# nyu-dl/MultimodalGame

Measured on AMD Instinct MI355X. Metric: exchange-steps/sec (whole node), 30-class Adaptive max_exchange=10 bs=64, higher is better.
Workload: dtype f32

## Files before the change

### multimodalgame_amd/csrc/kernels_bwd.h

```cpp
#pragma once
#include <type_traits>
#include "device_utils.h"
#include "layout.h"

namespace mmg {

template <bool CC = false>
__device__ __forceinline__ float combine_score(const float* part, size_t row, int npb, float b2) {
    float v = 0.f;
    if (npb <= 8) {
        float p[8];
#pragma unroll
        for (int j = 0; j < 8; ++j) p[j] = (j < npb) ? (CC ? __hip_atomic_load(&part[row * npb + j], __ATOMIC_RELAXED, __HIP_MEMORY_SCOPE_AGENT) : part[row * npb + j]) : 0.f;
#pragma unroll
        for (int j = 0; j < 8; ++j) v += p[j];
    } else {
        for (int j = 0; j < npb; ++j) v += part[row * npb + j];
    }
    return v + b2;
}

__host__ __device__ inline size_t partll_at(const Dims& d, int sen_side, size_t row, int npb) { return ((size_t)(sen_side ? 0 : 1) * d.T * d.B + row) * npb; }
__device__ __forceinline__ float combine_score_ll(const Dims& dm, const Tape& tp, int sen_side, size_t row, int npb, float b2, uint32_t epoch, bool need) {
    const size_t at = partll_at(dm, sen_side, row, npb);
// ... 396 lines not shown
            __syncthreads();
        }
        if (binary) {
            const float wh = (L - tp.bs[row]) * cw_z[t];
            for (int j = tid; j < W; j += nt) {
                const float v = bit_seed(tp.z[row * W + j], tp.pz[row * W + j], wh, ce_z[t]);
                s_dlz[j] = v; tp.dlz[row * W + j] = v;
            }
            __syncthreads();
            gemv_t<TU>(P.p[S_BIN_W], H, W, H, s_dlz, s_da, s_red, false);
            for (int i = tid; i < H; i += nt) {
                const float a = tp.a[row * H + i];
                const float v = s_da[i] * (1.f - a * a);
                s_dpre[i] = v; tp.dpre[row * H + i] = v; s_dhx[i] += v;
            }
            __syncthreads();
            if (t == 0) {
                gemv_t<TU>(P.p[S_CODE_W], W, H, W, s_dpre, s_dc0, s_red, false);
                for (int j = tid; j < W; j += nt) tp.dc0[(size_t)b * W + j] = s_dc0[j];
            }
            const float dbs = lc.cb[t] * (tp.bs[row] - L), dbr = lc.cb[t] * (tp.br[row] - L);
            if (tid == 0) { tp.dbs[row] = dbs; tp.dbr[row] = dbr; }
        } else {
            for (int i = tid; i < W; i += nt) tp.dlz[row * W + i] = 0.f;
            for (int i = tid; i < H; i += nt) tp.dpre[row * H + i] = 0.f;
            if (tid == 0) { tp.dbs[row] = 0.f; tp.dbr[row] = 0.f; }
        }
        __syncthreads();
    }
    for (int i = tid; i < H; i += nt) tp.dhx[(size_t)b * H + i] = s_dhx[i];
    if (!binary) for (int j = tid; j < W; j += nt) tp.dc0[(size_t)b * W + j] = 0.f;
}

template <bool CC = false>
__device__ __forceinline__ void build_row_map(const Dims& dm, const Tape& tp) {
    const int lane = threadIdx.x & 63, B = dm.B, T = dm.T;
    int base = 0;
    for (int t = 0; t < T; ++t) {
        for (int b0 = 0; b0 < B; b0 += 64) {
            const int b = b0 + lane;
            const int tsb = CC ? __hip_atomic_load(&tp.tstar[min(b, B - 1)], __ATOMIC_RELAXED, __HIP_MEMORY_SCOPE_AGENT) : tp.tstar[min(b, B - 1)];
            const bool act = (b < B) && (t <= tsb);
            const unsigned long long m = __ballot(act);
            const int pos = base + __popcll(m & ((1ull << lane) - 1ull));
            if (act) tp.rmap[pos] = t * B + b;
            base += __popcll(m);
        }
    }
    if (lane == 0) tp.rcount[0] = base;
    for (int i = base + lane; i < T * B; i += 64) tp.rmap[i] = -1;
}

template <bool CC = false>
__device__ __forceinline__ void dC_class(const Dims& dm, const Params& P, const Tape& tp, int d, float* s_c, float* s_p) {
    auto ld = [](const float* p) { return CC ? __hip_atomic_load(p, __ATOMIC_RELAXED, __HIP_MEMORY_SCOPE_AGENT) : *p; };
    const int tid = threadIdx.x, R = dm.R, B = dm.B, D = dm.D;
    const int cols = R < 64 ? R : 64;
    const int groups = MMG_BLOCK / cols;
    const int g = tid / cols, rr = tid - g * cols;
    const float* w2 = P.p[R_Y2_W];
    for (int r0 = 0; r0 < R; r0 += cols) {
        const int r = r0 + rr;
        float dc0 = 0.f, dc1 = 0.f, py0 = 0.f, py1 = 0.f;
        if (g < groups && r < R) {
            const float cv = ld(&tp.Cd[(size_t)d * R + r]);
            for (int b = g; b < B; b += 16 * groups) {
                float yv[16], pv[16];
#pragma unroll
                for (int u = 0; u < 16; ++u) {
                    const int bb = b + u * groups;
                    const bool ok = bb < B;
                    yv[u] = ok ? ld(&tp.dy[(size_t)bb * D + d]) : 0.f;
                    pv[u] = ok ? ld(&tp.Astar[(size_t)bb * R + r]) + cv : 0.f;
                }
#pragma unroll
                for (int u = 0; u < 16; u += 2) {
                    if (pv[u] > 0.f) { dc0 += yv[u]; py0 = fmaf(yv[u], pv[u], py0); }
                    if (pv[u + 1] > 0.f) { dc1 += yv[u + 1]; py1 = fmaf(yv[u + 1], pv[u + 1], py1); }
                }
            }
        }
        s_c[tid] = (dc0 + dc1) * ((g < groups && r < R) ? w2[r] : 0.f);
        s_p[tid] = py0 + py1;
        __syncthreads();
        if (tid < cols && r0 + tid < R) {
            float a = 0.f, c = 0.f;
            for (int k = 0; k < groups; ++k) { a += s_c[k * cols + tid]; c += s_p[k * cols + tid]; }
            tp.dC[(size_t)d * R + r0 + tid] = a;
            tp.Py2[(size_t)d * R + r0 + tid] = c;
        }
        __syncthreads();
    }
}

__global__ __launch_bounds__(MMG_BLOCK) void k_dC(Dims dm, Params P, Tape tp) {
    __shared__ float s_c[MMG_BLOCK], s_p[MMG_BLOCK];
    dC_class(dm, P, tp, blockIdx.x, s_c, s_p);
}

enum { SRC_STATIC = 0, SRC_X = 1, SRC_DESC = 2 };
struct GemmJob { const float* A; const float* Bm; float* C; const float* vhid; const float* vw2;
                 int lda, ldb, ldc, rows, N, K, bmod, bsrc, tile_begin, tiles_k, compact, nsplit; };
struct ColJob { const float* src; float* dst; const float* scale; const float* vbeta; const float* vw2; const float* wrow;
                int ld, rows, cols, blk_begin, compact, special; };
#define MMG_MAX_GEMM 40
#define MMG_MAX_COL 40
struct NormPlan { int64_t begin[MMG_GN_BLOCKS], end[MMG_GN_BLOCKS]; int agent[MMG_GN_BLOCKS]; };
#define MMG_MAX_WBLOCKS 16384
struct JobTable {
    int n_gemm, n_col, gemm_tiles, gemm_blocks, col_blocks, special_block, special_job, pad2;
    GemmJob g[MMG_MAX_GEMM];
    ColJob c[MMG_MAX_COL];
    NormPlan np;
    int g_begin[64], c_begin[64];
    int n_wblocks;
    signed char wblock_agent[MMG_MAX_WBLOCKS];
};

__device__ __forceinline__ float4 load4_guard(const float* __restrict__ base_, size_t row_off, int col, int ncols, bool row_ok, bool vec_ok) {
    float4 v = make_float4(0.f, 0.f, 0.f, 0.f);
    if (!row_ok) return v;
    gfloat* p = as_global(base_) + row_off + col;
    if (vec_ok && col + 3 < ncols) return ldg4(p);
    if (col < ncols) v.x = p[0];
    if (col + 1 < ncols) v.y = p[1];
    if (col + 2 < ncols) v.z = p[2];
    if (col + 3 < ncols) v.w = p[3];
    return v;
}

struct WgHead { int gemm_tiles, n_wblocks, special_block, special_job; };

struct OptArgs {
    int optim_type, only_receiver, from_wgrad, bump_step, bump_mb;
    float lr;
    int64_t agent_begin[5];
    int64_t total;
};

struct WgOpt {
    OptArgs oa;
    float* params; float* state; const float* grads; float* gnll; float* coefll;
    uint32_t* counter; uint32_t* err_host;
};
#define MMG_COEF_REPL 64
__device__ __forceinline__ void opt_update_one(const OptArgs& oa, float* params, float* state, int64_t idx, float g, float coef,
                                               float w, float s1, float s2, uint32_t step) {
    const float gv = g * coef;
    if (oa.optim_type == MMG_OPT_RMSPROP) {
        const float sv = 0.99f * s1 + (1.f - 0.99f) * gv * gv;
        w -= oa.lr * gv / (sqrtf(sv) + 1e-8f);
        state[idx] = sv;
    } else if (oa.optim_type == MMG_OPT_ADAM) {
        const float b1 = 0.9f, b2 = 0.999f;
        const float bc1 = 1.f - powf(b1, (float)step), bc2s = sqrtf(1.f - powf(b2, (float)step));
        const float mv = s1 + (gv - s1) * (1.f - b1), vv = b2 * s2 + (1.f - b2) * gv * gv;
        w -= (oa.lr / bc1) * mv / (sqrtf(vv) / bc2s + 1e-8f);
        state[idx] = mv; state[oa.total + idx] = vv;
    } else {
        w -= oa.lr * gv;
    }
    params[idx] = w;
}
__device__ __forceinline__ float opt_wait_coef(const WgOpt& wo, int agent, uint32_t epoch, const uint32_t* sync) {
    unsigned long long u;
    for (int spins = 0;; ) {
        u = ld_ll(wo.coefll, (size_t)agent * MMG_COEF_REPL + (blockIdx.x & (MMG_COEF_REPL - 1)));
        if (ll_fresh(u, epoch)) break;
        __builtin_amdgcn_s_sleep(2);
        if (++spins > (1 << 20)) { __hip_atomic_store(const_cast<uint32_t*>(sync) + MMG_SYNC_ERR, 10u, __ATOMIC_RELAXED, __HIP_MEMORY_SCOPE_AGENT); return -1.f; }
    }
    return ll_value(u);
}

template <bool OPT>
__global__ __launch_bounds__(MMG_BLOCK) void k_wgrad(const JobTable* __restrict__ jt, const float* __restrict__ x,
                                                     const float* __restrict__ desc, float* __restrict__ part,
                                                     Dims dm, const double* __restrict__ stats, float* __restrict__ losses,
                                                     double* __restrict__ totals, const int* __restrict__ rmap,
                                                     const int* __restrict__ rcount, float* __restrict__ wpart, uint32_t* __restrict__ wcnt,
                                                     const uint32_t* __restrict__ sync, float* __restrict__ grad_tail, WgOpt wo, int gt_stride, WgHead hd
#ifdef MMG_TIMING
                                                     , long long* __restrict__ dbg2
#endif
                                                     ) {
    const int bid = (gt_stride > 0 && (int)blockIdx.x >= gt_stride) ? (int)blockIdx.x - gt_stride + hd.gemm_tiles : (int)blockIdx.x;
    const uint32_t oepoch = OPT ? wo.counter[3] + 1u : 0u;
    const uint32_t ostep = OPT ? wo.counter[1] + 1u : 0u;
    if (OPT && bid > hd.n_wblocks) {
        __shared__ float s_ss[4];
        const int agent = bid - hd.n_wblocks - 1;
        const int n = hd.n_wblocks;
        float ss = 0.f;
        for (int k0 = threadIdx.x; k0 < n; k0 += 8 * MMG_BLOCK) {
            unsigned long long u[8]; bool mine[8], any[8];
#pragma unroll
            for (int q = 0; q < 8; ++q) {
                const int k = k0 + q * MMG_BLOCK;
                mine[q] = (k < n) && ((int)jt->wblock_agent[min(k, n - 1)] == agent);
                any[q] = __any(mine[q]);
                u[q] = 0ull;
            }
            for (int spins = 0;; ) {
                bool fresh = true;
#pragma unroll
                for (int q = 0; q < 8; ++q)
                    if (any[q]) {
                        const unsigned long long v = ld_ll(wo.gnll, (size_t)min(k0 + q * MMG_BLOCK, n - 1));
                        if (mine[q]) { u[q] = v; fresh = fresh && ll_fresh(v, oepoch); }
                    }
                if (!__any(!fresh)) break;
                __builtin_amdgcn_s_sleep(1);
                if (++spins > (1 << 20)) { __hip_atomic_store(const_cast<uint32_t*>(sync) + MMG_SYNC_ERR, 11u, __ATOMIC_RELAXED, __HIP_MEMORY_SCOPE_AGENT); break; }
            }
#pragma unroll
            for (int q = 0; q < 8; ++q) ss += mine[q] ? ll_value(u[q]) : 0.f;
        }
        const float wsum = dpp_wave_sum(ss);
        if ((threadIdx.x & 63) == 0) s_ss[threadIdx.x >> 6] = wsum;
        __syncthreads();
        const uint32_t err = __hip_atomic_load(sync + MMG_SYNC_ERR, __ATOMIC_RELAXED, __HIP_MEMORY_SCOPE_AGENT);
        if (threadIdx.x < MMG_COEF_REPL + 1) {
            const float tot = (s_ss[0] + s_ss[1]) + (s_ss[2] + s_ss[3]);
            const float coef = 1.0f / (sqrtf(tot) + 1e-6f);
            if (threadIdx.x < MMG_COEF_REPL) st_ll(wo.coefll, (size_t)agent * MMG_COEF_REPL + threadIdx.x, err != 0u ? -1.f : (coef < 1.f ? coef : 1.f), oepoch);
            else st_ll(wo.coefll, (size_t)4 * MMG_COEF_REPL + agent, tot, oepoch);
        }
        return;
    }
#ifdef MMG_TIMING
    if (threadIdx.x == 0 && blockIdx.x < 4096) dbg2[2 * blockIdx.x] = (long long)wall_clock64();
#define MMG_WG_END() do { __syncthreads(); if (threadIdx.x == 0 && blockIdx.x < 4096) dbg2[2 * blockIdx.x + 1] = (long long)wall_clock64(); } while (0)
#else
#define MMG_WG_END() do {} while (0)
#endif
    constexpr int CH = 64;
    __shared__ __attribute__((aligned(16))) float s_a[2][CH][16];
    __shared__ __attribute__((aligned(16))) float s_b[2][CH][48];
    float (*s_acc)[16][33] = reinterpret_cast<float (*)[16][33]>(&s_b[0][0][0]);
    float* s_part = &s_b[0][0][0];
    __shared__ float s_red[8];
    if (bid == hd.special_block) {
        const ColJob& C = jt->c[hd.special_job];
        float* s_v = &s_b[0][0][0];
        const int Hh = C.ld, Wc = C.cols, nb = C.rows;
        const int p8 = threadIdx.x & 7, jj = threadIdx.x >> 3;
        float wreg[32];
        const bool wfast = (Hh == 256) && (Wc <= 32);
        if (wfast) {
#pragma unroll
            for (int i = 0; i < 32; ++i) wreg[i] = C.wrow[(size_t)(p8 + 8 * i) * Wc + min(jj, Wc - 1)];
        }
        for (int h0 = threadIdx.x; h0 < Hh; h0 += MMG_BLOCK) {
            float a0 = 0.f, a1 = 0.f, a2 = 0.f, a3 = 0.f;
            for (int b0 = 0; b0 < nb; b0 += 64) {
                float v[64];
#pragma unroll
                for (int u = 0; u < 64; ++u) v[u] = C.src[(size_t)min(b0 + u, nb - 1) * Hh + h0];
#pragma unroll
                for (int u = 0; u < 64; u += 4) {
                    a0 += (b0 + u < nb) ? v[u] : 0.f; a1 += (b0 + u + 1 < nb) ? v[u + 1] : 0.f;
                    a2 += (b0 + u + 2 < nb) ? v[u + 2] : 0.f; a3 += (b0 + u + 3 < nb) ? v[u + 3] : 0.f;
                }
            }
            s_v[h0] = (a0 + a1) + (a2 + a3);
        }
        __syncthreads();
        float sq = 0.f;
        for (int j0 = 0; j0 < Wc; j0 += MMG_BLOCK / 8) {
            const int j = j0 + jj;
            float acc = 0.f;
            if (wfast) {
#pragma unroll
                for (int i = 0; i < 32; ++i) acc = fmaf(wreg[i], s_v[p8 + 8 * i], acc);
            } else if (j < Wc) {
                for (int h0 = p8; h0 < Hh; h0 += 8) acc = fmaf(C.wrow[(size_t)h0 * Wc + j], s_v[h0], acc);
            }
            acc = dpp_group_sum<8>(acc);
            if (j < Wc && p8 == 0) { const float gsum = acc * C.scale[j]; C.dst[j] = gsum; sq = fmaf(gsum, gsum, sq); }
        }
        sq = block_sum(sq, s_red);
        if (threadIdx.x == 0) part[bid] = sq;
        if (OPT) {
            if (threadIdx.x == 0) st_ll(wo.gnll, bid, sq, oepoch);
#ifdef MMG_TIMING
        if (threadIdx.x == 0 && bid < 2000) dbg2[8192 + 4 * bid + 2] = (long long)wall_clock64();
#endif
#ifdef MMG_TIMING
            if (threadIdx.x == 0 && bid < 2000) dbg2[8192 + 4 * bid + 2] = (long long)wall_clock64();
#endif
            const float coef = opt_wait_coef(wo, jt->wblock_agent[bid], oepoch, sync);
            for (int j0 = 0; j0 < Wc && coef >= 0.f; j0 += MMG_BLOCK / 8) {
                const int j = j0 + jj;
                if (j < Wc && p8 == 0) {
                    const int64_t idx = (C.dst - wo.grads) + j;
                    opt_update_one(wo.oa, wo.params, wo.state, idx, C.dst[j], coef, wo.params[idx], wo.state[idx],
                                   wo.oa.optim_type == MMG_OPT_ADAM ? wo.state[wo.oa.total + idx] : 0.f, ostep);
                }
            }
        }
        MMG_WG_END();
        return;
    }
    constexpr int MAXMAP = 2048;
    __shared__ unsigned short s_map[MAXMAP];
    const bool use_map = rmap != nullptr;
    int nact = 0;
    if (use_map) {
        const int tb = dm.T * dm.B;
        for (int i2 = threadIdx.x; i2 < tb; i2 += MMG_BLOCK) s_map[i2] = (unsigned short)rmap[i2];
        nact = rcount[0];
    }
    const int lane = threadIdx.x & 63, wave = threadIdx.x >> 6;
    if (bid == hd.n_wblocks) {
        float* s_lc = &s_b[0][0][0];
        LossCoef lc; lc.cw = s_lc; lc.ce = s_lc + 3 * dm.T; lc.cb = s_lc + 6 * dm.T;
        loss_coefficients(dm, stats, lc, losses, totals, !OPT);
        if (threadIdx.x == 0) {
            grad_tail[0] = (__hip_atomic_load(sync + MMG_SYNC_ERR, __ATOMIC_RELAXED, __HIP_MEMORY_SCOPE_AGENT) != 0u) ? 1.f : 0.f;
            grad_tail[1] = (float)stats[stat_glob(dm.T, 0)];
            grad_tail[2] = (float)stats[stat_glob(dm.T, 1)];
            grad_tail[3] = 0.f;
        }
        if (OPT) {
            __shared__ float s_tot[4];
            if (threadIdx.x < 4) {
                unsigned long long u;
                for (int spins = 0;; ) {
                    u = ld_ll(wo.coefll, (size_t)4 * MMG_COEF_REPL + threadIdx.x);
                    if (ll_fresh(u, oepoch)) break;
                    __builtin_amdgcn_s_sleep(2);
                    if (++spins > (1 << 20)) { __hip_atomic_store(const_cast<uint32_t*>(sync) + MMG_SYNC_ERR, 11u, __ATOMIC_RELAXED, __HIP_MEMORY_SCOPE_AGENT); break; }
                }
                s_tot[threadIdx.x] = ll_value(u);
            }
            __syncthreads();
            if (threadIdx.x == 0) {
                bool bad = false;
#pragma unroll
                for (int a = 0; a < 4; ++a) bad = bad || !(s_tot[a] == s_tot[a]) || s_tot[a] > 3.0e38f;
                losses[0] = bad ? __builtin_nanf("") : (float)(-stats[stat_glob(dm.T, 0)] / (double)dm.Bg);
                const uint32_t err = __hip_atomic_load(sync + MMG_SYNC_ERR, __ATOMIC_RELAXED, __HIP_MEMORY_SCOPE_AGENT);
                if (wo.err_host && (err != 0u || *wo.err_host == 0u)) *wo.err_host = err;
                if (err == 0u) wo.counter[2] = ostep;
                if (wo.oa.bump_mb) { wo.counter[0] += 1u; wo.counter[3] += 1u; }
            }
        }
        return;
    }
    if (bid < hd.gemm_tiles) {
      __shared__ int s_arrived;
      for (int vt = bid; vt < hd.gemm_tiles; vt += (gt_stride > 0 ? gt_stride : hd.gemm_tiles)) {
        const int nwg = hd.gemm_tiles, xq = nwg >> 3, xr = nwg & 7;
        const int xcd = vt & 7, slot = vt >> 3;
        const int tile = (xcd < xr ? xcd * (xq + 1) : xr * (xq + 1) + (xcd - xr) * xq) + slot;
        const int j = __popcll(__ballot(jt->g_begin[lane] <= tile)) - 1;
        const GemmJob& G = jt->g[j];
        const int ns = G.nsplit > 1 ? G.nsplit : 1;
        const int lts = tile - G.tile_begin, sp = lts % ns, lt = lts / ns;
        const int tn = lt / G.tiles_k, tk = lt - tn * G.tiles_k;
        const int n0 = tn * 16, k0 = tk * 32;
        const int i = lane & 15, q = lane >> 4;
        const float* Bbase = (G.bsrc == SRC_X) ? x : (G.bsrc == SRC_DESC) ? desc : G.Bm;
        const bool virt = G.vhid != nullptr;
        const float* Abase = virt ? G.vhid : G.A;
        const bool cmp = use_map && G.compact;
        const int lda = G.lda, ldb = G.ldb, bmod = G.bmod, N = G.N, K = G.K;
        const bool ident0 = cmp && dm.B >= 64 && sp == 0;
        int rows = cmp ? 0 : G.rows;
        const bool veca = ((lda & 3) == 0) && ((((uintptr_t)Abase) & 15) == 0);
        const bool vecb = ((ldb & 3) == 0) && ((((uintptr_t)Bbase) & 15) == 0);
        const int la = threadIdx.x >> 2, lac = (threadIdx.x & 3) * 4;
        const int lb0 = threadIdx.x >> 3, lbc = (threadIdx.x & 7) * 4;
        float4 vw = make_float4(0.f, 0.f, 0.f, 0.f);
        if (virt) vw = load4_guard(G.vw2, 0, n0 + lac, N, true, false);
        int nchunks_all = 0, cps = 0, cbeg = 0, cend = 0, nchunks = 0, rows_end = 0, rlast = 0;
        auto set_rows = [&](int r) {
            rows = r;
            nchunks_all = (rows + CH - 1) / CH; cps = (nchunks_all + ns - 1) / ns;
            cbeg = sp * cps; cend = min(nchunks_all, cbeg + cps); nchunks = max(cend - cbeg, 0);
            rows_end = min(rows, cend * CH);
            rlast = rows - 1;
        };
        if (!cmp) set_rows(G.rows);
        constexpr int DEPTH = 3;
        f32x4 acc0 = {0.f, 0.f, 0.f, 0.f}, acc1 = {0.f, 0.f, 0.f, 0.f};
        const bool interior = veca && vecb && ((G.bsrc != SRC_X) || (k0 + 32 <= K));
        const int bmodv = bmod ? bmod : 0x7fffffff;
        const uint32_t bmagic = bmod > 1 ? (uint32_t)((0x100000000ull + (unsigned)bmod - 1ull) / (unsigned)bmod) : 0u;
        const bool bmod_one = bmod == 1;
        (void)bmodv;
        auto rowmod = [&](int r) -> int {
            const int q = (int)__umulhi((uint32_t)r, bmagic);
            const int m = r - q * bmod;
            return bmod_one ? 0 : (m < 0 ? m + bmod : m);
        };
        gfloat* const Ag = as_global(Abase);
        gfloat* const Bg = as_global(Bbase);
        gfloat* const betag = as_global(G.A);
        auto run = [&](auto virt_tag, auto cmp_tag, auto bmod_tag) {
            constexpr bool VIRT = decltype(virt_tag)::value, CMPJ = decltype(cmp_tag)::value, BMOD = decltype(bmod_tag)::value;
            float4 ra[DEPTH], rb0[DEPTH], rb1[DEPTH];
            float beta[DEPTH];
            const uint32_t acol = (uint32_t)(n0 + lac), bcol = (uint32_t)(k0 + lbc), ulda = (uint32_t)lda, uldb = (uint32_t)ldb;
            auto issue = [&](int rc_, int c0_, int c1_, int u) {
                ra[u] = ldg4(Ag + ((uint32_t)rc_ * ulda + acol));
                if (VIRT) beta[u] = betag[(uint32_t)rc_];
                rb0[u] = ldg4(Bg + ((uint32_t)(BMOD ? rowmod(c0_) : c0_) * uldb + bcol));
                rb1[u] = ldg4(Bg + ((uint32_t)(BMOD ? rowmod(c1_) : c1_) * uldb + bcol));
            };
            auto fetch = [&](int c, int u) {
                const int r_ = c * CH + la, r0_ = c * CH + lb0, r1_ = r0_ + 32;
                int rc_ = min(r_, rlast), c0_ = min(r0_, rlast), c1_ = min(r1_, rlast);
                if (CMPJ) { rc_ = s_map[rc_]; c0_ = s_map[c0_]; c1_ = s_map[c1_]; }
                issue(rc_, c0_, c1_, u);
            };
            if (!CMPJ) {
#pragma unroll
                for (int u = 0; u < DEPTH - 1; ++u) fetch(cbeg + u, u);
            } else if (ident0) issue(la, lb0, lb0 + 32, 0);
            if (use_map) __syncthreads();
#ifdef MMG_TIMING
            if (threadIdx.x == 0 && tile < 2000) dbg2[8192 + 4 * tile + 0] = (long long)wall_clock64();
#endif
            if (CMPJ) {
                set_rows(nact);
#pragma unroll
                for (int u = 0; u < DEPTH - 1; ++u) if (u > 0 || !ident0) fetch(cbeg + u, u);
            }
            const int nouter = (nchunks + DEPTH - 1) / DEPTH;
            for (int o = 0; o < nouter; ++o) {
#pragma unroll
                for (int u = 0; u < DEPTH; ++u) {
                    const int c = cbeg + o * DEPTH + u;
                    const int buf = (o * DEPTH + u) & 1;
                    const bool va = (c * CH + la) < rows_end;
                    float4 av = ra[u];
                    if (VIRT) {
                        av.x = av.x > 0.f ? beta[u] * vw.x : 0.f; av.y = av.y > 0.f ? beta[u] * vw.y : 0.f;
                        av.z = av.z > 0.f ? beta[u] * vw.z : 0.f; av.w = av.w > 0.f ? beta[u] * vw.w : 0.f;
                    }
                    const float ma = va ? 1.f : 0.f;
                    *reinterpret_cast<float4*>(&s_a[buf][la][lac]) = make_float4(av.x * ma, av.y * ma, av.z * ma, av.w * ma);
                    *reinterpret_cast<float4*>(&s_b[buf][lb0][lbc]) = rb0[u];
                    *reinterpret_cast<float4*>(&s_b[buf][lb0 + 32][lbc]) = rb1[u];
                    __syncthreads();
                    fetch(c + DEPTH - 1, (u + DEPTH - 1) % DEPTH);
#pragma unroll
                    for (int v = 0; v < 4; ++v) {
                        const int r = wave * 16 + v * 4 + q;
                        const float a = s_a[buf][r][i];
                        acc0 = mfma16(a, s_b[buf][r][i], acc0);
                        acc1 = mfma16(a, s_b[buf][r][16 + i], acc1);
                    }
                }
            }
        };
        auto run_b = [&](auto virt_tag, auto cmp_tag) {
            if (bmod != 0) run(virt_tag, cmp_tag, std::true_type{}); else run(virt_tag, cmp_tag, std::false_type{});
        };
        auto run_c = [&](auto virt_tag) { if (cmp) run_b(virt_tag, std::true_type{}); else run_b(virt_tag, std::false_type{}); };
        if (interior) {
            if (virt) run_c(std::true_type{}); else run_c(std::false_type{});
        } else {
            if (use_map) __syncthreads();
            if (cmp) set_rows(nact);
            for (int c = cbeg; c < cend; ++c) {
                const int buf = c & 1;
                const int rl = c * CH + la;
                const bool rv = rl < rows_end;
                const int r = cmp ? (int)s_map[min(rl, rlast)] : rl;
                float4 av = load4_guard(Abase, (size_t)(rv ? r : 0) * lda, n0 + lac, N, rv, veca);
                if (virt) {
                    const float be = rv ? betag[r] : 0.f;
                    av.x = av.x > 0.f ? be * vw.x : 0.f; av.y = av.y > 0.f ? be * vw.y : 0.f;
                    av.z = av.z > 0.f ? be * vw.z : 0.f; av.w = av.w > 0.f ? be * vw.w : 0.f;
                }
                const int r0l = c * CH + lb0, r1l = r0l + 32;
                const bool v0 = r0l < rows_end, v1 = r1l < rows_end;
                const int r0 = cmp ? (int)s_map[min(r0l, rlast)] : r0l, r1 = cmp ? (int)s_map[min(r1l, rlast)] : r1l;
                const int m0 = bmod ? (r0 % bmod) : r0, m1 = bmod ? (r1 % bmod) : r1;
                const float4 b0v = load4_guard(Bbase, (size_t)(v0 ? m0 : 0) * ldb, k0 + lbc, K, v0, vecb);
                const float4 b1v = load4_guard(Bbase, (size_t)(v1 ? m1 : 0) * ldb, k0 + lbc, K, v1, vecb);
                *reinterpret_cast<float4*>(&s_a[buf][la][lac]) = av;
                *reinterpret_cast<float4*>(&s_b[buf][lb0][lbc]) = b0v;
                *reinterpret_cast<float4*>(&s_b[buf][lb0 + 32][lbc]) = b1v;
                __syncthreads();
#pragma unroll
                for (int v = 0; v < 4; ++v) {
                    const int rr2 = wave * 16 + v * 4 + q;
                    const float a = s_a[buf][rr2][i];
                    acc0 = mfma16(a, s_b[buf][rr2][i], acc0);
                    acc1 = mfma16(a, s_b[buf][rr2][16 + i], acc1);
                }
            }
        }
        __syncthreads();
#ifdef MMG_TIMING
        if (threadIdx.x == 0 && tile < 2000) dbg2[8192 + 4 * tile + 1] = (long long)wall_clock64();
#endif
#pragma unroll
        for (int r = 0; r < 4; ++r) { s_acc[wave][q * 4 + r][i] = acc0[r]; s_acc[wave][q * 4 + r][16 + i] = acc1[r]; }
        __syncthreads();
        float sq = 0.f;
        float gv2[2]; int64_t gi2[2];
#pragma unroll
        for (int h2 = 0; h2 < 2; ++h2) {
            const int rr = threadIdx.x >> 4, cc = (threadIdx.x & 15) + 16 * h2;
            const int n = n0 + rr, k = k0 + cc;
            const float v = (s_acc[0][rr][cc] + s_acc[1][rr][cc]) + (s_acc[2][rr][cc] + s_acc[3][rr][cc]);
            gv2[h2] = v; gi2[h2] = -1;
            if (ns > 1) st_wt(&wpart[(size_t)tile * 512 + rr * 32 + cc], v);
            else if (n < N && k < K) {
                as_global_w(G.C)[(size_t)n * G.ldc + k] = v;
                sq = fmaf(v, v, sq);
                gi2[h2] = (G.C - wo.grads) + (int64_t)n * G.ldc + k;
            }
        }
        bool adds_up = false;
        if (ns > 1) {
            asm volatile("s_waitcnt vmcnt(0)" ::: "memory");
            __syncthreads();
            const int tile0 = tile - sp;
            if (threadIdx.x == 0) s_arrived = (int)__hip_atomic_fetch_add(wcnt + tile0, 1u, __ATOMIC_RELAXED, __HIP_MEMORY_SCOPE_AGENT);
            __syncthreads();
            adds_up = __builtin_amdgcn_readfirstlane(s_arrived) == ns - 1;
            if (adds_up) {
                if (threadIdx.x == 0) __hip_atomic_store(wcnt + tile0, 0u, __ATOMIC_RELAXED, __HIP_MEMORY_SCOPE_AGENT);
#pragma unroll
                for (int h2 = 0; h2 < 2; ++h2) {
                    const int rr = threadIdx.x >> 4, cc = (threadIdx.x & 15) + 16 * h2;
                    float v = 0.f;
                    for (int s0 = 0; s0 < ns; s0 += 8) {
                        float pv[8];
#pragma unroll
                        for (int u = 0; u < 8; ++u) pv[u] = ld_cc(&wpart[(size_t)(tile0 + min(s0 + u, ns - 1)) * 512 + rr * 32 + cc]);
#pragma unroll
                        for (int u = 0; u < 8; ++u) v += (s0 + u < ns) ? pv[u] : 0.f;
                    }
                    const int n = n0 + rr, k = k0 + cc;
                    if (n < N && k < K) { as_global_w(G.C)[(size_t)n * G.ldc + k] = v; sq = fmaf(v, v, sq); }
                }
            }
        }
        sq = block_sum(sq, s_red);
        if (threadIdx.x == 0) {
            if (ns == 1) part[tile] = sq;
            else {
                if (sp != 0) part[tile] = 0.f;
                if (adds_up) part[tile - sp] = sq;
            }
        }
        if (OPT) {
            if (threadIdx.x == 0) st_ll(wo.gnll, tile, sq, oepoch);
            float w[2], s1[2], s2[2];
#pragma unroll
            for (int h2 = 0; h2 < 2; ++h2) {
                const int64_t ic = gi2[h2] >= 0 ? gi2[h2] : 0;
                w[h2] = wo.params[ic]; s1[h2] = wo.state[ic];
                s2[h2] = (wo.oa.optim_type == MMG_OPT_ADAM) ? wo.state[wo.oa.total + ic] : 0.f;
            }
#ifdef MMG_TIMING
            if (threadIdx.x == 0 && tile < 2000) dbg2[8192 + 4 * tile + 2] = (long long)wall_clock64();
#endif
            const float coef = opt_wait_coef(wo, jt->wblock_agent[tile], oepoch, sync);
#ifdef MMG_TIMING
            if (threadIdx.x == 0 && tile < 2000) dbg2[8192 + 4 * tile + 3] = (long long)wall_clock64();
#endif
            if (coef >= 0.f) {
#pragma unroll
                for (int h2 = 0; h2 < 2; ++h2)
                    if (gi2[h2] >= 0) opt_update_one(wo.oa, wo.params, wo.state, gi2[h2], gv2[h2], coef, w[h2], s1[h2], s2[h2], ostep);
            }
        }
        __syncthreads();
      }
        MMG_WG_END();
        return;
    }
    const int cb = bid - hd.gemm_tiles;
    const int j = __popcll(__ballot(jt->c_begin[lane] <= cb)) - 1;
    const ColJob& C = jt->c[j];
    const bool ccmp = use_map && C.compact;
    if (use_map) __syncthreads();
    const int c0 = (cb - C.blk_begin) * 16;
    const int rows = ccmp ? nact : C.rows, ld = C.ld;
    const bool virt = C.vbeta != nullptr;
    const bool wsum = C.wrow != nullptr;
    gfloat* const rowv = as_global(virt ? C.vbeta : wsum ? C.wrow : C.src);
    const bool vec4 = (c0 + 16 <= C.cols) && !(ld & 3) && !(((uintptr_t)(C.src + c0)) & 15) && rows > 0;
    int ngroups = 16;
    if (vec4) {
        ngroups = 64;
        const int cq = (threadIdx.x & 3) * 4, g = threadIdx.x >> 2;
        gfloat* const sp = as_global(C.src) + (c0 + cq);
        float4 vw = make_float4(0.f, 0.f, 0.f, 0.f);
        if (virt) vw = make_float4(C.vw2[c0 + cq], C.vw2[c0 + cq + 1], C.vw2[c0 + cq + 2], C.vw2[c0 + cq + 3]);
        float4 A0 = make_float4(0.f, 0.f, 0.f, 0.f), A1 = A0;
        constexpr int UN = 8;
        const int rlast = rows - 1;
        for (int r0 = g; r0 < rows; r0 += 64 * UN) {
            float4 hv[UN]; float bv[UN];
#pragma unroll
            for (int u = 0; u < UN; ++u) {
                const int rl = min(r0 + 64 * u, rlast);
                const int r = ccmp ? (int)s_map[rl] : rl;
                hv[u] = ldg4(sp + (size_t)r * ld);
                bv[u] = rowv[(virt || wsum) ? r : 0];
            }
#pragma unroll
            for (int u = 0; u < UN; ++u) {
                const bool ok = (r0 + 64 * u) < rows;
                float4& A = (u & 1) ? A1 : A0;
                if (wsum) {
                    const float w = ok ? bv[u] : 0.f;
                    A.x = fmaf(hv[u].x, w, A.x); A.y = fmaf(hv[u].y, w, A.y); A.z = fmaf(hv[u].z, w, A.z); A.w = fmaf(hv[u].w, w, A.w);
                } else if (virt) {
                    const float w = ok ? bv[u] : 0.f;
                    A.x += hv[u].x > 0.f ? w * vw.x : 0.f; A.y += hv[u].y > 0.f ? w * vw.y : 0.f;
                    A.z += hv[u].z > 0.f ? w * vw.z : 0.f; A.w += hv[u].w > 0.f ? w * vw.w : 0.f;
                } else {
                    A.x += ok ? hv[u].x : 0.f; A.y += ok ? hv[u].y : 0.f; A.z += ok ? hv[u].z : 0.f; A.w += ok ? hv[u].w : 0.f;
                }
            }
        }
        *reinterpret_cast<float4*>(&s_part[g * 16 + cq]) = make_float4(A0.x + A1.x, A0.y + A1.y, A0.z + A1.z, A0.w + A1.w);
    } else {
        const int ncol = min(16, C.cols - c0);
        const int lp = ncol > 8 ? 4 : ncol > 4 ? 3 : ncol > 2 ? 2 : ncol > 1 ? 1 : 0, P = 1 << lp, NG = MMG_BLOCK >> lp;
        const int cc = threadIdx.x & (P - 1), g = threadIdx.x >> lp;
        const bool cv = cc < ncol;
        float a0 = 0.f, a1 = 0.f, a2 = 0.f, a3 = 0.f;
        if (cv) {
            const float* sp = C.src + c0 + cc;
            constexpr int UN = 16;
            const float vw = virt ? C.vw2[c0 + cc] : 0.f;
            for (int r0 = g; r0 < rows; r0 += NG * UN) {
                float hv[UN], bv[UN];
#pragma unroll
                for (int u = 0; u < UN; ++u) {
                    const int rl = r0 + NG * u;
                    const bool ok = rl < rows;
                    const int r = (ccmp && ok) ? (int)s_map[rl] : rl;
                    hv[u] = ok ? sp[(size_t)r * ld] : 0.f;
                    bv[u] = (ok && (virt || wsum)) ? rowv[r] : 0.f;
                }
#pragma unroll
                for (int u = 0; u < UN; u += 4) {
                    if (wsum) {
                        a0 = fmaf(hv[u], bv[u], a0); a1 = fmaf(hv[u + 1], bv[u + 1], a1);
                        a2 = fmaf(hv[u + 2], bv[u + 2], a2); a3 = fmaf(hv[u + 3], bv[u + 3], a3);
                    } else if (virt) {
                        a0 += hv[u] > 0.f ? bv[u] * vw : 0.f; a1 += hv[u + 1] > 0.f ? bv[u + 1] * vw : 0.f;
                        a2 += hv[u + 2] > 0.f ? bv[u + 2] * vw : 0.f; a3 += hv[u + 3] > 0.f ? bv[u + 3] * vw : 0.f;
                    } else {
                        a0 += hv[u]; a1 += hv[u + 1]; a2 += hv[u + 2]; a3 += hv[u + 3];
                    }
                }
            }
        }
        float av = (a0 + a1) + (a2 + a3);
        for (int off = 32; off >= P; off >>= 1) av += __shfl_xor(av, off);
        ngroups = 4;
        if ((threadIdx.x & 63) < P) s_part[(threadIdx.x >> 6) * 16 + cc] = av;
    }
    __syncthreads();
    float v = 0.f;
    if (threadIdx.x < 16 && (c0 + (int)threadIdx.x) < C.cols) {
        for (int k = 0; k < ngroups; ++k) v += s_part[k * 16 + threadIdx.x];
        if (C.scale) v *= C.scale[c0 + threadIdx.x];
        C.dst[c0 + threadIdx.x] = v;
    }
    const float sq = block_sum(v * v, s_red);
    if (threadIdx.x == 0) part[bid] = sq;
    if (OPT) {
        if (threadIdx.x == 0) st_ll(wo.gnll, bid, sq, oepoch);
        const bool mine = threadIdx.x < 16 && (c0 + (int)threadIdx.x) < C.cols;
        const int64_t idx = mine ? (C.dst - wo.grads) + c0 + threadIdx.x : 0;
        const float w = wo.params[idx], s1 = wo.state[idx], s2 = (wo.oa.optim_type == MMG_OPT_ADAM) ? wo.state[wo.oa.total + idx] : 0.f;
        const float coef = opt_wait_coef(wo, jt->wblock_agent[bid], oepoch, sync);
        if (coef >= 0.f && mine) opt_update_one(wo.oa, wo.params, wo.state, idx, v, coef, w, s1, s2, ostep);
    }
    MMG_WG_END();
}

__global__ __launch_bounds__(MMG_BLOCK) void k_gradnorm(const JobTable* __restrict__ jt, const float* __restrict__ grads,
                                                        float* __restrict__ part, uint32_t* __restrict__ counter,
                                                        const float* __restrict__ grad_tail, float* __restrict__ losses,
                                                        double* __restrict__ totals, int fix_bg) {
    __shared__ float s_red[8];
    const int blk = blockIdx.x;
    const int64_t b0 = jt->np.begin[blk], b1 = jt->np.end[blk];
    float acc = 0.f;
    for (int64_t i = b0 + (int64_t)threadIdx.x * 4; i < b1; i += (int64_t)blockDim.x * 4) {
        const float4 g = *reinterpret_cast<const float4*>(grads + i);
        acc = fmaf(g.x, g.x, acc); acc = fmaf(g.y, g.y, acc); acc = fmaf(g.z, g.z, acc); acc = fmaf(g.w, g.w, acc);
    }
    acc = block_sum(acc, s_red);
    if (threadIdx.x == 0) {
        part[blk] = acc;
        if (blk == 0) counter[1] += 1u;
        if (blk == 0 && fix_bg > 0) {
            const float hits = grad_tail[2];
            totals[1] += (double)hits - (double)losses[7];
            losses[0] = -grad_tail[1] / (float)fix_bg;
            losses[7] = hits;
        }
    }
}


__global__ __launch_bounds__(MMG_BLOCK) void k_opt(const JobTable* __restrict__ jt, OptArgs oa, float* __restrict__ params,
                                                   const float* __restrict__ grads, float* __restrict__ state,
                                                   const float* __restrict__ part, const uint32_t* __restrict__ counter,
                                                   const uint32_t* __restrict__ sync, uint32_t* __restrict__ err_host,
                                                   const float* __restrict__ grad_tail, float* __restrict__ losses) {
    uint32_t err = __hip_atomic_load(sync + MMG_SYNC_ERR, __ATOMIC_RELAXED, __HIP_MEMORY_SCOPE_AGENT);
    if (err == 0u && grad_tail && grad_tail[0] != 0.f) err = MMG_SYNC_ERR_REMOTE;
    if (oa.bump_mb && blockIdx.x == 0 && threadIdx.x == 0) { const_cast<uint32_t*>(counter)[0] += 1u; const_cast<uint32_t*>(counter)[3] += 1u; }
    if (err_host && blockIdx.x == 0 && threadIdx.x == 0 && (err != 0u || *err_host == 0u)) *err_host = err;
    if (err != 0u) return;
    __shared__ float s_coef[4];
    __shared__ float s_ss[4][4];
    float* st1 = state; float* st2 = state + oa.total;
    const int64_t i0 = ((int64_t)blockIdx.x * blockDim.x + threadIdx.x) * 4;
    const bool have = i0 < oa.total;
    const int64_t il = have ? i0 : 0;
    const float4 g0 = *reinterpret_cast<const float4*>(grads + il);
    const float4 w0 = *reinterpret_cast<const float4*>(params + il);
    const float4 s0 = *reinterpret_cast<const float4*>(st1 + il);
    const float4 v0 = (oa.optim_type == MMG_OPT_ADAM) ? *reinterpret_cast<const float4*>(st2 + il) : make_float4(0.f, 0.f, 0.f, 0.f);
    const uint32_t step = counter[1] + (oa.bump_step ? 1u : 0u);
    {
        const int n = oa.from_wgrad ? jt->n_wblocks : MMG_GN_BLOCKS;
        float ss[4] = {0.f, 0.f, 0.f, 0.f};
        for (int k0 = threadIdx.x; k0 < n; k0 += 8 * MMG_BLOCK) {
            float v[8]; int a[8];
#pragma unroll
            for (int u = 0; u < 8; ++u) {
                const int k = k0 + u * MMG_BLOCK;
                const bool ok = k < n;
                v[u] = ok ? part[k] : 0.f;
                a[u] = ok ? (oa.from_wgrad ? (int)jt->wblock_agent[k] : jt->np.agent[k]) : -1;
            }
#pragma unroll
            for (int u = 0; u < 8; ++u) {
                ss[0] += (a[u] == 0) ? v[u] : 0.f; ss[1] += (a[u] == 1) ? v[u] : 0.f;
                ss[2] += (a[u] == 2) ? v[u] : 0.f; ss[3] += (a[u] == 3) ? v[u] : 0.f;
            }
        }
#pragma unroll
        for (int a = 0; a < 4; ++a) {
            const float wsum = dpp_wave_sum(ss[a]);
            if ((threadIdx.x & 63) == 0) s_ss[a][threadIdx.x >> 6] = wsum;
        }
        __syncthreads();
        if (threadIdx.x < 4) {
            const float tot = (s_ss[threadIdx.x][0] + s_ss[threadIdx.x][1]) + (s_ss[threadIdx.x][2] + s_ss[threadIdx.x][3]);
            const float norm = sqrtf(tot);
            const float coef = 1.0f / (norm + 1e-6f);
            s_coef[threadIdx.x] = coef < 1.f ? coef : 1.f;
            if (losses && blockIdx.x == 0 && (!(tot == tot) || tot > 3.0e38f)) losses[0] = __builtin_nanf("");
        }
    }
    __syncthreads();
    const float b1 = 0.9f, b2 = 0.999f;
    float bc1 = 1.f, bc2s = 1.f;
    if (oa.optim_type == MMG_OPT_ADAM) {
        bc1 = 1.f - powf(b1, (float)step);
        bc2s = sqrtf(1.f - powf(b2, (float)step));
    }
    for (int64_t i = i0; i < oa.total; i += (int64_t)gridDim.x * blockDim.x * 4) {
        int a = 0;
        if (i >= oa.agent_begin[1]) a = 1;
        if (i >= oa.agent_begin[2]) a = 2;
        if (i >= oa.agent_begin[3]) a = 3;
        if (oa.only_receiver && a != 0) continue;
        const float coef = s_coef[a];
        const bool first = (i == i0);
        float4 g = first ? g0 : *reinterpret_cast<const float4*>(grads + i);
        float4 w = first ? w0 : *reinterpret_cast<float4*>(params + i);
        float gv[4] = {g.x * coef, g.y * coef, g.z * coef, g.w * coef};
        float wv[4] = {w.x, w.y, w.z, w.w};
        if (oa.optim_type == MMG_OPT_RMSPROP) {
            float4 sq = first ? s0 : *reinterpret_cast<float4*>(st1 + i);
            float sv[4] = {sq.x, sq.y, sq.z, sq.w};
#pragma unroll
            for (int k = 0; k < 4; ++k) {
                sv[k] = 0.99f * sv[k] + (1.f - 0.99f) * gv[k] * gv[k];
                wv[k] -= oa.lr * gv[k] / (sqrtf(sv[k]) + 1e-8f);
            }
            *reinterpret_cast<float4*>(st1 + i) = make_float4(sv[0], sv[1], sv[2], sv[3]);
        } else if (oa.optim_type == MMG_OPT_ADAM) {
            float4 m = first ? s0 : *reinterpret_cast<float4*>(st1 + i), v = first ? v0 : *reinterpret_cast<float4*>(st2 + i);
            float mv[4] = {m.x, m.y, m.z, m.w}, vv[4] = {v.x, v.y, v.z, v.w};
#pragma unroll
            for (int k = 0; k < 4; ++k) {
                mv[k] = mv[k] + (gv[k] - mv[k]) * (1.f - b1);
                vv[k] = b2 * vv[k] + (1.f - b2) * gv[k] * gv[k];
                const float denom = sqrtf(vv[k]) / bc2s + 1e-8f;
                wv[k] -= (oa.lr / bc1) * mv[k] / denom;
            }
            *reinterpret_cast<float4*>(st1 + i) = make_float4(mv[0], mv[1], mv[2], mv[3]);
            *reinterpret_cast<float4*>(st2 + i) = make_float4(vv[0], vv[1], vv[2], vv[3]);
        } else {
#pragma unroll
            for (int k = 0; k < 4; ++k) wv[k] -= oa.lr * gv[k];
        }
        *reinterpret_cast<float4*>(params + i) = make_float4(wv[0], wv[1], wv[2], wv[3]);
    }
    if (oa.bump_step && blockIdx.x == gridDim.x - 1) {
        __syncthreads();
        if (threadIdx.x == 0) const_cast<uint32_t*>(counter)[2] = step;
    }
}


__host__ __device__ inline int64_t log_snapshot_count(int T, int B, int W, int k, bool with_losses) {
    return (with_losses ? 8 + 1 + (int64_t)stat_count(T) + T + 2 * (int64_t)B : 0) + (k > 0 ? (int64_t)T + 4 * (int64_t)T * k * W + 2 * (int64_t)T * k : 0);
}
__global__ __launch_bounds__(MMG_BLOCK) void k_log_snapshot(Dims dm, Tape tp, const int64_t* __restrict__ target, int k, int with_losses, double* __restrict__ out) {
    __shared__ float s_red[8];
    const int T = dm.T, B = dm.B, D = dm.D, W = dm.W, tid = threadIdx.x, lane = tid & 63, wave = tid >> 6;
    const int nst = stat_count(T);
    const int64_t o_ent = 9 + nst, o_arg = o_ent + T, o_tgt = o_arg + B, o_dump = with_losses ? o_tgt + B : 0;
    const int blk = blockIdx.x;
    if (blk < T) {
        if (!with_losses) return;
        float acc = 0.f;
        for (int b = wave; b < B; b += MMG_BLOCK / 64) {
            const float* yr = tp.y + ((size_t)blk * B + b) * D;
            float m = -3.0e38f;
            for (int d = lane; d < D; d += 64) m = fmaxf(m, yr[d]);
            m = wave_max(m);
            float se = 0.f;
            for (int d = lane; d < D; d += 64) se += __expf(yr[d] - m);
            se = wave_sum(se);
            const float inv = 1.0f / se;
            float e = 0.f;
            for (int d = lane; d < D; d += 64) { const float p = __expf(yr[d] - m) * inv; e += p * __logf(p + 1e-8f); }
            acc += wave_sum(e);
        }
        if (lane == 0) s_red[wave] = acc;
        __syncthreads();
        if (tid == 0) out[o_ent + blk] = (double)(((s_red[0] + s_red[1]) + (s_red[2] + s_red[3])) / (float)B);
        return;
    }
    if (blk == T) {
        if (!with_losses) return;
        if (tid < 8) out[tid] = (double)tp.losses[tid];
        if (tid == 8) out[8] = tp.totals[1];
        for (int i = tid; i < nst; i += MMG_BLOCK) out[9 + i] = tp.stats[i];
        for (int b = tid; b < B; b += MMG_BLOCK) {
            const float* dr = tp.dist + (size_t)b * D;
            float best = dr[0]; int arg = 0;
            for (int d = 1; d < D; ++d) { const float v = dr[d]; if (v > best) { best = v; arg = d; } }
            out[o_arg + b] = (double)arg;
            out[o_tgt + b] = target ? (double)target[b] : 0.0;
        }
        return;
    }
    if (k <= 0) return;
    double* od = out + o_dump;
    for (int t = wave; t < T; t += MMG_BLOCK / 64) {
        float a = 0.f;
        for (int b = lane; b < B; b += 64) a += (float)tp.mask[(size_t)(t + 1) * B + b];
        a = wave_sum(a);
        if (lane == 0) od[t] = (double)a;
    }
    const int64_t nW = (int64_t)T * k * W;
    const float* src[4] = {tp.pz, tp.pw, tp.z, tp.w};
#pragma unroll
    for (int a = 0; a < 4; ++a)
        for (int64_t i = tid; i < nW; i += MMG_BLOCK) {
            const int t = (int)(i / ((int64_t)k * W)), r = (int)(i % ((int64_t)k * W)), b = r / W, j = r % W;
            od[T + a * nW + i] = (double)src[a][((size_t)t * B + b) * W + j];
        }
    for (int i = tid; i < T * k; i += MMG_BLOCK) {
        const int t = i / k, b = i % k;
        od[T + 4 * nW + i] = (double)tp.ps[(size_t)t * B + b];
        od[T + 4 * nW + T * k + i] = (double)tp.mask[(size_t)(t + 1) * B + b];
    }
}

}
```

Before: 127,700.

## Overlap row-map and job-table loads with first GEMM fetches in backward kernel

The row-map staging into LDS and the job-table lookup are hoisted before the branch. They are issued as register loads together with the first tile's job lookup, and the LDS stores are deferred until after the GEMM prefetch loads have been issued. This hides the latency of those global loads behind the tile's initial operand fetches instead of serialising them at block start. Job descriptors are also copied by value, and an explicit waitcnt is added before the barrier in the optimiser path. The cost is extra register pressure from holding up to MAXMAP/MMG_BLOCK list values per thread and more complex control flow.

```diff
diff --git a/multimodalgame_amd/csrc/kernels_bwd.h b/multimodalgame_amd/csrc/kernels_bwd.h
--- a/multimodalgame_amd/csrc/kernels_bwd.h
+++ b/multimodalgame_amd/csrc/kernels_bwd.h
@@ -722,15 +722,6 @@
         MMG_WG_END();
         return;
     }
-    constexpr int MAXMAP = 2048;
-    __shared__ unsigned short s_map[MAXMAP];
-    const bool use_map = rmap != nullptr;
-    int nact = 0;
-    if (use_map) {
-        const int tb = dm.T * dm.B;
-        for (int i2 = threadIdx.x; i2 < tb; i2 += MMG_BLOCK) s_map[i2] = (unsigned short)rmap[i2];
-        nact = rcount[0];
-    }
     const int lane = threadIdx.x & 63, wave = threadIdx.x >> 6;
     if (bid == hd.n_wblocks) {
         float* s_lc = &s_b[0][0][0];
@@ -768,14 +759,59 @@
         }
         return;
     }
-    if (bid < hd.gemm_tiles) {
+    auto tile_of = [&](int vt) {
+        const int nwg = hd.gemm_tiles, xq = nwg >> 3, xr = nwg & 7;
+        const int xcd = vt & 7, slot = vt >> 3;
+        return (xcd < xr ? xcd * (xq + 1) : xr * (xq + 1) + (xcd - xr) * xq) + slot;
+    };
+    constexpr int MAXMAP = 2048;
+    __shared__ unsigned short s_map[MAXMAP];
+    const bool use_map = rmap != nullptr;
+    const bool is_gemm = bid < hd.gemm_tiles;
+    const int tb = dm.T * dm.B;
+    const int first_blk = is_gemm ? tile_of(bid) : bid - hd.gemm_tiles;
+    const int* const lk = is_gemm ? jt->g_begin : jt->c_begin;
+    int begin_l, j0, nact = 0, nact_v = 0;
+    int lv[MAXMAP / MMG_BLOCK];
+    auto lookup_and_list = [&](auto nl_tag) {
+        constexpr int NL = decltype(nl_tag)::value;
+        int lkl = lane;
+        asm volatile("; job lookup, list variant %1" : "+v"(lkl) : "n"(NL));
+        begin_l = lk[lkl];
+#pragma unroll
+        for (int q = 0; q < NL; ++q) lv[q] = rmap[min((int)threadIdx.x + q * MMG_BLOCK, tb - 1)];
+        if (NL > 0) {
+            int zl = 0;
+            asm volatile("; live-row count: a vector load" : "+v"(zl));
+            nact_v = rcount[zl];
+        }
+        asm volatile("; job lookup landed, %1 list loads in flight" : "+v"(begin_l) : "n"(NL));
+        j0 = __popcll(__ballot(begin_l <= first_blk)) - 1;
+    };
+    const bool short_list = tb <= 3 * MMG_BLOCK;
+    if (use_map) {
+        if (short_list) lookup_and_list(std::integral_constant<int, 3>{});
+        else lookup_and_list(std::integral_constant<int, MAXMAP / MMG_BLOCK>{});
+    } else lookup_and_list(std::integral_constant<int, 0>{});
+    bool list_pending = use_map;
+    auto store_list = [&]() {
+        if (!list_pending) return;
+        list_pending = false;
+        nact = __builtin_amdgcn_readfirstlane(nact_v);
+        if (short_list) {
+#pragma unroll
+            for (int q = 0; q < 3; ++q) s_map[(int)threadIdx.x + q * MMG_BLOCK] = (unsigned short)lv[q];
+        } else {
+#pragma unroll
+            for (int q = 0; q < MAXMAP / MMG_BLOCK; ++q) s_map[(int)threadIdx.x + q * MMG_BLOCK] = (unsigned short)lv[q];
+        }
+    };
+    if (is_gemm) {
       __shared__ int s_arrived;
       for (int vt = bid; vt < hd.gemm_tiles; vt += (gt_stride > 0 ? gt_stride : hd.gemm_tiles)) {
-        const int nwg = hd.gemm_tiles, xq = nwg >> 3, xr = nwg & 7;
-        const int xcd = vt & 7, slot = vt >> 3;
-        const int tile = (xcd < xr ? xcd * (xq + 1) : xr * (xq + 1) + (xcd - xr) * xq) + slot;
-        const int j = __popcll(__ballot(jt->g_begin[lane] <= tile)) - 1;
-        const GemmJob& G = jt->g[j];
+        const int tile = vt == bid ? first_blk : tile_of(vt);
+        const int j = vt == bid ? j0 : __popcll(__ballot(begin_l <= tile)) - 1;
+        const GemmJob G = jt->g[j];
         const int ns = G.nsplit > 1 ? G.nsplit : 1;
         const int lts = tile - G.tile_begin, sp = lts % ns, lt = lts / ns;
         const int tn = lt / G.tiles_k, tk = lt - tn * G.tiles_k;
@@ -838,7 +874,9 @@
             if (!CMPJ) {
 #pragma unroll
                 for (int u = 0; u < DEPTH - 1; ++u) fetch(cbeg + u, u);
-            } else if (ident0) issue(la, lb0, lb0 + 32, 0);
+                store_list();
+            } else if (ident0) { issue(la, lb0, lb0 + 32, 0); store_list(); }
+            else store_list();
             if (use_map) __syncthreads();
 #ifdef MMG_TIMING
             if (threadIdx.x == 0 && tile < 2000) dbg2[8192 + 4 * tile + 0] = (long long)wall_clock64();
@@ -883,6 +921,7 @@
         if (interior) {
             if (virt) run_c(std::true_type{}); else run_c(std::false_type{});
         } else {
+            store_list();
             if (use_map) __syncthreads();
             if (cmp) set_rows(nact);
             for (int c = cbeg; c < cend; ++c) {
@@ -993,15 +1032,16 @@
                     if (gi2[h2] >= 0) opt_update_one(wo.oa, wo.params, wo.state, gi2[h2], gv2[h2], coef, w[h2], s1[h2], s2[h2], ostep);
             }
         }
+        if (OPT) __builtin_amdgcn_s_waitcnt(0x0F70);
         __syncthreads();
       }
         MMG_WG_END();
         return;
     }
     const int cb = bid - hd.gemm_tiles;
-    const int j = __popcll(__ballot(jt->c_begin[lane] <= cb)) - 1;
-    const ColJob& C = jt->c[j];
+    const ColJob C = jt->c[j0];
     const bool ccmp = use_map && C.compact;
+    store_list();
     if (use_map) __syncthreads();
     const int c0 = (cb - C.blk_begin) * 16;
     const int rows = ccmp ? nact : C.rows, ld = C.ld;
```

Result: faster. 129,800, median of 6 (+1.7%).
